# ChaissonLab/LRA

Hardware: AMD Instinct MI355X
Metric: aligned Gbp/s, 30 kb ONT vs GRCh38 (MapRead_lowacc end to end incl. SAM text), per job (higher is better)
Workload: dtype int32

## Files before the change

### lra_amd/csrc/aog.hip

```cpp
#include "common.h"
#include <stdlib.h>
#include <algorithm>
#include <vector>
#include <type_traits>

namespace {

constexpr int MISS = -(1 << 30);
enum { A_DONE = 0, A_LEFT = 1, A_DOWN = 2, A_DIAG = 3, A_BORDER = 4, A_GAPLEFT = 5, A_GAPDOWN = 6 };

constexpr int CLASS_A_BYTES = 10 * 1024;
constexpr int CLASS_B_BYTES = 64 * 1024;
constexpr int CLASS_M1_BYTES = 20 * 1024;
constexpr int CLASS_M2_BYTES = 32 * 1024;
constexpr int LN_MAX = 24, LN_ROWW = 2;
constexpr int LN_ARROW_WORDS = LN_MAX * LN_ROWW, LN_PREV_WORDS = LN_MAX + 2, LN_CODE_BYTES = LN_MAX + 1;
constexpr int LN_BYTES = 64 * (4 * LN_ARROW_WORDS + 4 * LN_PREV_WORDS + 2 * LN_CODE_BYTES);
constexpr int NCLS = 19;
constexpr int CLASS_S_BYTES = 2560;
constexpr long HBM_SLOT_BYTES = 4L << 20;
constexpr long HBM_SLOT_B_BYTES = 8L << 20;
constexpr int ROLL_WINDOW = 256;
constexpr int ROLL_CODE_BYTES = 4096;
constexpr int REG_S_BYTES = 2048, REG_M_BYTES = 8192, REG_L_BYTES = 32768;
constexpr int REG_L_USED = 16384;

__device__ __forceinline__ int code_n(unsigned char c) {
  if (c < 8) return c & 3;
  switch (c) {
    case 'A': case 'a': return 0;
    case 'C': case 'c': return 1;
    case 'G': case 'g': return 2;
    case 'T': case 't': return 3;
    default: return 4;
  }
}

struct Geo {
  int qLen, tLen, diag, k, R, qB, tB;
  bool top;
  int n;
  int nUsed;
};

__host__ __device__ __forceinline__ bool make_geo(int qLen, int tLen, int k0, Geo& g) {
  g.qLen = qLen; g.tLen = tLen;
  g.diag = max(1, min(qLen, tLen));
  int k = min(g.diag, k0);
  g.top = true;
  if (g.diag + 2 * k >= max(qLen, tLen)) { k *= 2; g.top = false; }
  g.k = k;
  g.R = 2 * k + 3;
  long n = (long)(3 + k + g.diag) * g.R;
  g.qB = min(g.diag + k, qLen + 1);
  g.tB = min(g.diag + k, tLen + 1);
  if (n > (1L << 28)) { g.n = 0; g.nUsed = 0; return false; }
  g.n = (int)n;
  g.nUsed = g.top ? g.n : min(g.n, g.tB * g.R);
  return true;
}

__host__ __device__ __forceinline__ long align4(long x) { return (x + 3) & ~3L; }

__host__ __device__ __forceinline__ long need_bytes(const Geo& g) {
  long suf = g.top ? (4L * g.n + align4(g.n)) : 0;
  return 4L * g.nUsed + align4(g.nUsed) + suf + 16L * (g.diag + 1) + align4(g.qLen + 1) + align4(g.tLen + 1);
}

__host__ __device__ __forceinline__ long need_bytes_reg(const Geo& g) { return align4(g.nUsed) + align4(g.qLen + 1) + align4(g.tLen + 1); }

struct Shape { int qLen, tLen, k0; };
struct Scoring { int m, mm, indel; };
template <typename P, typename S>
__host__ __device__ __forceinline__ bool problem_ok(const P& pr, const S& a, Geo& g) {
  bool ok = pr.qLen >= 0 && pr.tLen >= 0 && pr.k0 >= 1 && make_geo(pr.qLen, pr.tLen, pr.k0, g);
  long mx = max(abs(a.m), max(abs(a.mm), abs(a.indel)));
  return ok && ((long)(pr.qLen + pr.tLen + 16) * (mx + 1) < (1L << 28));
}

__host__ __device__ __forceinline__ int class_of(const Geo& g) {
  const long need = need_bytes(g);
  int cls = need <= CLASS_A_BYTES ? 0 : need <= CLASS_M1_BYTES ? 4 : need <= CLASS_M2_BYTES ? 5 : need <= CLASS_B_BYTES ? 1 : 2;
  if (g.k + 1 <= 32) cls = cls == 0 ? 7 : cls == 4 ? 8 : cls == 5 ? 9 : cls;
  if (need <= CLASS_S_BYTES && g.k + 1 <= 16) cls = 3;
  if (cls == 2 && need > HBM_SLOT_BYTES) cls = 6;
  if (cls == 6 && need > HBM_SLOT_B_BYTES) return -1;
  if (!g.top) {
    const long nr = need_bytes_reg(g);
    if (g.qLen <= LN_MAX && g.tLen <= LN_MAX) { const int mx = max(g.qLen, g.tLen); cls = mx <= 3 ? 14 : mx <= 6 ? 15 : mx <= 10 ? 16 : mx <= 16 ? 17 : 18; }
    else if (g.k + 2 <= 16 && nr <= REG_S_BYTES) cls = 10;
    else if (g.k + 2 <= 32 && nr <= REG_M_BYTES) cls = 11;
    else if (g.k + 2 <= 64 && nr <= REG_L_USED) cls = 12;
  }
  return cls;
}

__host__ __device__ __forceinline__ bool hbm_codes_in_lds(const Geo& g) { return g.qLen + g.tLen + 2 <= ROLL_CODE_BYTES; }
__host__ __device__ __forceinline__ bool hbm_in_regs(const Geo& g, int G) { return g.k + 2 <= G; }
__host__ __device__ __forceinline__ bool hbm_rolling(const Geo& g, int G) { return !g.top && (hbm_in_regs(g, G) || (2 * g.k + 3 <= ROLL_WINDOW && hbm_codes_in_lds(g))); }

__host__ __device__ __forceinline__ int path_of(const Geo& g, int cls) {
  int path = g.top ? LRA_AOG_PATH_SUFFIX : 0;
  if (cls == 2 || cls == 6) {
    const bool rolling = hbm_rolling(g, 64);
    path |= !rolling ? LRA_AOG_PATH_SCORES_HBM : hbm_in_regs(g, 64) ? LRA_AOG_PATH_SCORES_REGS : LRA_AOG_PATH_SCORES_ROLLING;
    if (rolling && hbm_codes_in_lds(g)) path |= LRA_AOG_PATH_CODES_LDS;
  } else {
    path |= (cls >= 10 && cls <= 12) ? LRA_AOG_PATH_SCORES_REGS : LRA_AOG_PATH_SCORES_LDS;
    path |= LRA_AOG_PATH_CODES_LDS;
  }
  return path;
}

struct Work {
  int* sPre; int* sSuf; int* loMax; int* loIdx; int* upMax; int* upIdx;
  signed char* pPre; signed char* pSuf; unsigned char* qc; unsigned char* tc;
};

template <typename BytePtr>
__device__ __forceinline__ Work carve(BytePtr base, const Geo& g) {
  Work w;
  auto* p = base;
  w.sPre = (int*)p; p += 4L * g.nUsed;
  w.sSuf = (int*)p; if (g.top) p += 4L * g.n;
  w.loMax = (int*)p; p += 4L * (g.diag + 1);
  w.loIdx = (int*)p; p += 4L * (g.diag + 1);
  w.upMax = (int*)p; p += 4L * (g.diag + 1);
  w.upIdx = (int*)p; p += 4L * (g.diag + 1);
  w.pPre = (signed char*)p; p += align4(g.nUsed);
  w.pSuf = (signed char*)p; if (g.top) p += align4(g.n);
  w.qc = (unsigned char*)p; p += align4(g.qLen + 1);
  w.tc = (unsigned char*)p;
  return w;
}

__device__ __forceinline__ void wave_sync() {
  __builtin_amdgcn_fence(__ATOMIC_RELEASE, "workgroup");
  __builtin_amdgcn_wave_barrier();
  __builtin_amdgcn_fence(__ATOMIC_ACQUIRE, "workgroup");
}

__device__ __forceinline__ void wave_sync_lds() {
  __builtin_amdgcn_fence(__ATOMIC_RELEASE, "wavefront");
  __builtin_amdgcn_wave_barrier();
  __builtin_amdgcn_fence(__ATOMIC_ACQUIRE, "wavefront");
}

struct Problem {
  const char* q; const char* t;
  int qLen, tLen, k0, m, mm, indel;
};

__device__ __forceinline__ int dpp_from_prev_lane(int v) { return __builtin_amdgcn_update_dpp(MISS, v, 0x138, 0xf, 0xf, false); }
__device__ __forceinline__ int dpp_from_next_lane(int v) { return __builtin_amdgcn_update_dpp(MISS, v, 0x130, 0xf, 0xf, false); }

template <int G, typename ArrowPtr, typename CodePtr>
__device__ __forceinline__ int reg_fill(int lane, int gbase, const Geo& g, int m, int mm, int indel, ArrowPtr P, CodePtr qc, CodePtr tc) {
  const int qLen = g.qLen, tLen = g.tLen, k = g.k, R = g.R, diag = g.diag, qB = g.qB, tB = g.tB;
  auto pre = [&](int i, int j) -> int {
    int v = MISS;
    if (j == 0 && i >= 1 && i < k + 1) v = indel * i;
    if (i == 0 && j >= 1 && j <= k + 1) v = indel * j;
    if (i == 0 && j == 0) v = 0;
    if (qLen >= tLen) { if (j == i + k + 1 && i <= diag - k - 1) v = MISS; if (i == j + k + 1 && j >= 1 && j < diag + k - 1) v = MISS; }
    if (qLen <= tLen) { if (i == j + k + 1 && j < diag - 1) v = MISS; if (j == i + k + 1 && j >= 1 && j < diag + k) v = MISS; }
    return v;
  };
  const int Wd = 2 * k + 3;
  const int sLast = max((qB - 1) + (tB - 1), 0);
  const int ci = qB - 1, cj = tB - 1;
  int vE = MISS, vO = MISS;
  const bool firstE = ((0 - k - 1) & 1) == 0;
  const int dE = 2 * lane - k - 1, dO = dE + 1;
  const bool okE = 2 * lane < Wd && dE >= -k && dE <= k, okO = 2 * lane + 1 < Wd && dO >= -k && dO <= k;
  const int sLoE = okE ? 2 + abs(dE) : INT_MAX, sHiE = min(2 * (qB - 1) - dE, 2 * (tB - 1) + dE);
  const int sLoO = okO ? 2 + abs(dO) : INT_MAX, sHiO = min(2 * (qB - 1) - dO, 2 * (tB - 1) + dO);
  const int s0E = firstE ? 0 : 1, s0O = firstE ? 1 : 0;
  int iE = (s0E + dE) >> 1, jE = s0E - iE, iO = (s0O + dO) >> 1, jO = s0O - iO;
  int adE = jE * R + 2 * lane, adO = jO * R + 2 * lane + 1;
  auto codes_match = [&](int i, int j) -> bool { return qc[min(max(i, 0), qLen)] == tc[min(max(j, 0), tLen)]; };
  bool eqE = codes_match(iE, jE), eqO = codes_match(iO, jO);
  auto step = [&](int s, auto isE) {
    constexpr bool E = decltype(isE)::value;
    const int nb1 = E ? dpp_from_prev_lane(vO) : dpp_from_next_lane(vE);
    const int i = E ? iE : iO, j = E ? jE : jO;
    const bool nxt = codes_match(i + 1, j + 1);
    int v = MISS;
    if (s >= (E ? sLoE : sLoO) && s <= (E ? sHiE : sHiO)) {
      const int sIns = (E ? nb1 : vE) + indel;
      const int sDel = (E ? vO : nb1) + indel;
      const int sMat = (E ? vE : vO) + ((E ? eqE : eqO) ? m : mm);
      const int best = max(sIns, max(sDel, sMat));
      v = best;
      P[E ? adE : adO] = (signed char)((best == sIns) ? A_LEFT : (best == sDel) ? A_DOWN : A_DIAG);
    } else if (s <= k + 1) {
      if (2 * lane + (E ? 0 : 1) < Wd && i >= 0 && j >= 0) v = pre(i, j);
    }
    if (E) { vE = v; eqE = nxt; iE++; jE++; adE += R; } else { vO = v; eqO = nxt; iO++; jO++; adO += R; }
  };
  int s = 0;
  bool lastE;
  if (firstE) {
    for (; s + 1 <= sLast; s += 2) { step(s, std::true_type{}); step(s + 1, std::false_type{}); }
    lastE = false;
    if (s <= sLast) { step(s, std::true_type{}); lastE = true; }
  } else {
    for (; s + 1 <= sLast; s += 2) { step(s, std::false_type{}); step(s + 1, std::true_type{}); }
    lastE = true;
    if (s <= sLast) { step(s, std::false_type{}); lastE = false; }
  }
  const int ddc = ci - cj + k + 1;
  const int corner = lastE ? vE : vO;
  return (ci >= 0 && cj >= 0 && ddc >= 0 && ddc < Wd && ((ddc & 1) == 0) == lastE) ? __shfl(corner, gbase + (ddc >> 1)) : MISS;
}

template <int G, typename BytePtr>
__device__ __forceinline__ void solve(int wlane, const Problem& pr, const Geo& g, BytePtr mem, int* out_score,
                      int* out_nb, int* blocks, long cap, int* out_status, int* roll = nullptr, int chunkBytes = 8192) {
  const int qLen = g.qLen, tLen = g.tLen, k = g.k, R = g.R, diag = g.diag, n = g.n, nUsed = g.nUsed;
  const int m = pr.m, mm = pr.mm, indel = pr.indel;
  const int lane = wlane & (G - 1), gbase = wlane - lane;
  Work w = carve(mem, g);
  int status = 0;
  auto PI = [&](int i, int j) { return j * R + (i - j) + k + 1; };
  auto inb = [&](int s) { return s >= 0 && s < n; };
#define PSET(slot, sc, ar)                                                         \
  do { int s__ = (slot); if (inb(s__)) { if (s__ < nUsed) { if (!rolling) w.sPre[s__] = (sc); w.pPre[s__] = (ar); } } else status |= LRA_ST_OOB_SLOT; } while (0)
#define SSET(slot, sc, ar)                                                         \
  do { int s__ = (slot); if (inb(s__)) { w.sSuf[s__] = (sc); w.pSuf[s__] = (ar); } else status |= LRA_ST_OOB_SLOT; } while (0)

  for (int x = lane; x <= qLen; x += G) w.qc[x] = x ? code_n((unsigned char)pr.q[x - 1]) : 0;
  for (int x = lane; x <= tLen; x += G) w.tc[x] = x ? code_n((unsigned char)pr.t[x - 1]) : 0;
  const bool codesInLds = hbm_codes_in_lds(g);
  const bool rolling = roll != nullptr && hbm_rolling(g, G);
  unsigned char* lq = (unsigned char*)(roll + 3 * ROLL_WINDOW); unsigned char* lt = lq + (qLen + 1);
  if (rolling && codesInLds) {
    for (int x = lane; x <= qLen; x += G) lq[x] = x ? code_n((unsigned char)pr.q[x - 1]) : 0;
    for (int x = lane; x <= tLen; x += G) lt[x] = x ? code_n((unsigned char)pr.t[x - 1]) : 0;
  }
  if (rolling) {
    const long head = min((long)nUsed, (long)((16 - ((uintptr_t)&w.pPre[0] & 15)) & 15));
    for (long x = lane; x < head; x += G) w.pPre[x] = -1;
    const long body = (nUsed - head) >> 4;
    int4* p16 = (int4*)(&w.pPre[0] + head);
    for (long x = lane; x < body; x += G) p16[x] = make_int4(-1, -1, -1, -1);
    for (long x = head + (body << 4) + lane; x < nUsed; x += G) w.pPre[x] = -1;
  }
  else for (int x = lane; x < nUsed; x += G) { w.sPre[x] = MISS; w.pPre[x] = -1; }
  if (g.top)
    for (int x = lane; x < n; x += G) { w.sSuf[x] = MISS; w.pSuf[x] = -1; }
  for (int x = lane; x <= diag; x += G) { w.loMax[x] = MISS; w.loIdx[x] = 0; w.upMax[x] = MISS; w.upIdx[x] = 0; }
  wave_sync();
  for (int i = 1 + lane; i < k + 1; i += G) PSET(PI(i, 0), indel * i, A_LEFT);
  for (int j = 1 + lane; j <= k + 1; j += G) PSET(PI(0, j), indel * j, A_DOWN);
  if (lane == 0) PSET(PI(0, 0), 0, A_DONE);
  wave_sync();
  if (qLen >= tLen) {
    for (int i = lane; i <= diag - k - 1; i += G) PSET(PI(i, i + k + 1), MISS, A_BORDER);
    for (int i = 1 + lane; i < diag + k - 1; i += G) PSET(PI(i + k + 1, i), MISS, A_BORDER);
  }
  if (qLen <= tLen) {
    for (int j = lane; j < diag - 1; j += G) PSET(PI(j + k + 1, j), MISS, A_BORDER);
    for (int j = 1 + lane; j < diag + k; j += G) PSET(PI(j - k - 1, j), MISS, A_BORDER);
  }
  wave_sync();
  const int qB = g.qB, tB = g.tB;
  int rollResult = MISS;
  if (rolling) {
    auto pre = [&](int i, int j) -> int {
      int v = MISS;
      if (j == 0 && i >= 1 && i < k + 1) v = indel * i;
      if (i == 0 && j >= 1 && j <= k + 1) v = indel * j;
      if (i == 0 && j == 0) v = 0;
      if (qLen >= tLen) { if (j == i + k + 1 && i <= diag - k - 1) v = MISS; if (i == j + k + 1 && j >= 1 && j < diag + k - 1) v = MISS; }
      if (qLen <= tLen) { if (i == j + k + 1 && j < diag - 1) v = MISS; if (j == i + k + 1 && j >= 1 && j < diag + k) v = MISS; }
      return v;
    };
    const int Wd = 2 * k + 3;
    const int sLast = (qB - 1) + (tB - 1);
    const bool inRegs = hbm_in_regs(g, G);
    if (inRegs) rollResult = codesInLds ? reg_fill<G>(lane, gbase, g, m, mm, indel, w.pPre, lq, lt) : reg_fill<G>(lane, gbase, g, m, mm, indel, w.pPre, w.qc, w.tc);
    for (int s = 0; !inRegs && s <= max(sLast, 0); s++) {
      int* cur = roll + (s % 3) * ROLL_WINDOW; const int* p1 = roll + ((s + 2) % 3) * ROLL_WINDOW; const int* p2 = roll + ((s + 1) % 3) * ROLL_WINDOW;
      int jlo = max(1, max(s - qB + 1, (s - k + 1) >> 1));
      if (s - k < 0) jlo = max(1, s - qB + 1);
      const int jhi = min(tB - 1, min(s - 1, (s + k) >> 1));
      for (int dd = lane; dd < Wd; dd += G) {
        const int d = dd - k - 1;
        int v = MISS;
        if (((s + d) & 1) == 0) {
          const int i = (s + d) >> 1, j = s - i;
          if (i >= 0 && j >= 0) {
            if (s >= 2 && j >= jlo && j <= jhi && d >= -k && d <= k) {
              const int sIns = p1[dd - 1] + indel, sDel = p1[dd + 1] + indel;
              const int sMat = p2[dd] + (lq[i] == lt[j] ? m : mm);
              const int best = max(sIns, max(sDel, sMat));
              const int ar = (best == sIns) ? A_LEFT : (best == sDel) ? A_DOWN : A_DIAG;
              v = best;
              w.pPre[PI(i, j)] = (signed char)ar;
            } else v = pre(i, j);
            if (i == qB - 1 && j == tB - 1) rollResult = v;
          }
        }
        cur[dd] = v;
      }
      wave_sync_lds();
    }
    wave_sync();
    if (!inRegs) { const int ddc = (qB - 1) - (tB - 1) + k + 1; rollResult = (ddc >= 0 && ddc < Wd) ? __shfl(rollResult, gbase + (ddc % G)) : MISS; }
  }
  for (int s = 2; !rolling && s <= (qB - 1) + (tB - 1); s++) {
    int jlo = max(1, max(s - qB + 1, (s - k + 1) >> 1));
    if (s - k < 0) jlo = max(1, s - qB + 1);
    int jhi = min(tB - 1, min(s - 1, (s + k) >> 1));
    for (int j = jlo + lane; j <= jhi; j += G) {
      int i = s - j;
      int sIns = w.sPre[PI(i - 1, j)] + indel;
      int sDel = w.sPre[PI(i, j - 1)] + indel;
      int sMat = w.sPre[PI(i - 1, j - 1)] + (w.qc[i] == w.tc[j] ? m : mm);
      int best = max(sIns, max(sDel, sMat));
      int ar = (best == sIns) ? A_LEFT : (best == sDel) ? A_DOWN : A_DIAG;
      int slot = PI(i, j);
      w.sPre[slot] = best;
      w.pPre[slot] = (signed char)ar;
    }
    wave_sync();
  }

  int ti, tj;
  int result;
  long nb = 0;
  const long iter_cap = 4L * (qLen + tLen + 8);
  int run = 0;
  auto flush = [&](int i_after, int j_after) {
    if (run > 0) {
      if (nb < cap) { blocks[3 * nb] = i_after; blocks[3 * nb + 1] = j_after; blocks[3 * nb + 2] = run; }
      else status |= LRA_ST_CAPACITY;
      nb++;
      run = 0;
    }
  };

  if (g.top) {
    for (int j = 1 + lane; j < tB && j <= diag; j += G) {
      int bm = MISS, bi = 0;
      int ihi = min(qB, j + k + 1);
      for (int i = max(1, j - k); i < ihi && i < qLen - k; i++) {
        int v = w.sPre[PI(i, j)];
        if (v >= bm) { bm = v; bi = i; }
      }
      w.loMax[j] = bm; w.loIdx[j] = bi;
    }
    for (int i = 1 + lane; i <= diag && i < qB; i += G) {
      int bm = MISS, bj = 0;
      int jhi = min(tB - 1, i + k);
      for (int j = max(1, i - k); j <= jhi && j < tLen; j++) {
        int v = w.sPre[PI(i, j)];
        if (v > bm) { bm = v; bj = j; }
      }
      w.upMax[i] = bm; w.upIdx[i] = bj;
    }
    if (lane == 0) {
      if (qLen >= tLen) { w.loMax[0] = 0; w.loIdx[0] = 0; }
      if (qLen <= tLen) { w.upMax[0] = 0; w.upIdx[0] = 0; }
    }
    wave_sync();
    const int qStart = max(0, qLen - diag);
    const int tStart = max(0, tLen - diag);
    const int tLow = max(0, tLen - diag - k - 1 - 1);
    const int qLow = max(0, qLen - diag - k - 1);
    const int tEnd = tLen + 1;
    auto SI = [&](int ii, int jj) {
      int a = ii - qLow, b = jj - tLow;
      return b * R + (a - b) + k + 1;
    };
    if (qLen >= tLen) {
      for (int i = qLow + lane; i < qStart + k + 1; i += G) SSET(SI(i, 0), w.loMax[0], A_GAPLEFT);
      wave_sync();
      for (int j = 1 + lane; j <= diag; j += G) SSET(SI(qLow + j - 1, j), w.loMax[j], A_GAPLEFT);
      wave_sync();
      for (int j = tStart + 1 + lane; j < tEnd - k; j += G) SSET(SI(qStart + (j - tStart - 1) + k + 1, j), MISS, A_BORDER);
      wave_sync();
    }
    if (qLen <= tLen) {
      for (int j = tLow + lane; j < tStart + k + 2; j += G) SSET(SI(qStart, j), w.upMax[0], A_GAPDOWN);
      wave_sync();
      for (int j = tStart + 1 + lane; j < tEnd; j += G) {
        int i = qStart + 1 + (j - tStart - 1);
        SSET(SI(i, j - k - 1), (i <= diag ? w.upMax[i] : MISS), A_GAPDOWN);
      }
      wave_sync();
      for (int j = tStart + lane; j < tEnd - k - 1; j += G) SSET(SI(qStart + (j - tStart), j + k + 1), MISS, A_BORDER);
      wave_sync();
    }
    const int c0 = qStart + diag - tLen;
    const bool qLong = qLen >= tLen;
    for (int s = (qLow + 1) + (tLow + 1); s <= qLen + tLen; s++) {
      int num = s - c0 - k;
      int jlo = (num >= 0) ? ((num + 1) >> 1) : -((-num) >> 1);
      jlo = max(jlo, max(tLow + 1, s - qLen));
      int num2 = s - c0 + k;
      int jhi = (num2 >= 0) ? (num2 >> 1) : -((-num2 + 1) >> 1);
      jhi = min(jhi, min(tLen, s - qLow - 1));
      for (int j = jlo + lane; j <= jhi; j += G) {
        int i = s - j;
        int delClose = MISS, insClose = MISS;
        if (qLong) delClose = (j <= diag) ? w.loMax[j] : MISS;
        else insClose = (i <= diag) ? w.upMax[i] : MISS;
        int a = SI(i - 1, j), b = SI(i, j - 1), c = SI(i - 1, j - 1);
        if (!inb(a) || !inb(b) || !inb(c)) { status |= LRA_ST_OOB_SLOT; continue; }
        int sIns = w.sSuf[a] + indel;
        int sDel = w.sSuf[b] + indel;
        int sMat = w.sSuf[c] + (w.qc[i] == w.tc[j] ? m : mm);
        int best = max(delClose, max(insClose, max(sIns, max(sDel, sMat))));
        int ar = (best == sIns) ? A_LEFT : (best == sDel) ? A_DOWN : (best == sMat) ? A_DIAG
                 : (best == delClose) ? A_GAPLEFT : A_GAPDOWN;
        SSET(SI(i, j), best, (signed char)ar);
      }
      wave_sync();
    }
    ti = qLen; tj = tLen;
    int s0 = SI(ti, tj);
    int arrow = inb(s0) ? w.pSuf[s0] : -1;
    result = inb(s0) ? w.sSuf[s0] : MISS;
    if (lane == 0) {
      long it = 0;
      while (arrow != A_DONE && arrow != A_GAPDOWN && arrow != A_GAPLEFT && ti >= 0 && tj >= 0) {
        if (++it > iter_cap) { status |= LRA_ST_NO_TERMINATION; break; }
        if (arrow == A_DIAG) { run++; ti--; tj--; }
        else if (arrow == A_LEFT) { flush(ti, tj); ti--; }
        else if (arrow == A_DOWN) { flush(ti, tj); tj--; }
        else { status |= LRA_ST_NO_TERMINATION; break; }
        if (ti >= 0 && tj >= 0) { int sl = SI(ti, tj); arrow = inb(sl) ? w.pSuf[sl] : -1; if (!inb(sl)) status |= LRA_ST_OOB_SLOT; }
      }
      flush(ti, tj);
      if (arrow == A_GAPDOWN && ti >= 0 && ti <= diag) tj = w.upIdx[ti];
      else if (arrow == A_GAPLEFT && tj >= 0 && tj <= diag) ti = w.loIdx[tj];
    }
  } else {
    ti = qB - 1; tj = tB - 1;
    result = rolling ? rollResult : w.sPre[PI(ti, tj)];
  }
  if (rolling) {
    unsigned char* chunk = (unsigned char*)(roll + 3 * ROLL_WINDOW + ROLL_CODE_BYTES / 4);
    const int chRows = max(1, chunkBytes / R);
    int cLo = 1, cHi = 0;
    auto arrowAt = [&](int i, int j) -> int {
      if (j < cLo || j > cHi) {
        cHi = j; cLo = max(0, j - chRows + 1);
        wave_sync();
        const long base = (long)cLo * R, len = (long)(cHi - cLo + 1) * R;
        for (long x = lane; x < len; x += G) chunk[x] = (unsigned char)w.pPre[base + x];
        wave_sync();
      }
      return (int)(signed char)chunk[(j - cLo) * R + (i - j) + k + 1];
    };
    auto flushL = [&](int i_after, int j_after) {
      if (run > 0) {
        if (nb < cap) { if (lane == 0) { blocks[3 * nb] = i_after; blocks[3 * nb + 1] = j_after; blocks[3 * nb + 2] = run; } }
        else status |= LRA_ST_CAPACITY;
        nb++;
        run = 0;
      }
    };
    constexpr int A_OFF = 100, A_WIN = 101;
    const unsigned long long gmask = (~0ULL >> (64 - G)) << gbase;
    if (ti >= 0 && tj >= 0 && inb(PI(ti, tj))) {
      while (true) {
        (void)arrowAt(ti, tj);
        const int jl = tj - lane;
        const bool on = ti - lane >= 0 && jl >= 0;
        const int a = !on ? A_OFF : jl < cLo ? A_WIN : (int)(signed char)chunk[(jl - cLo) * R + (ti - tj) + k + 1];
        const unsigned long long nd = (__ballot(a != A_DIAG) & gmask) >> gbase;
        const int f = nd ? __ffsll((long long)nd) - 1 : G;
        run += f; ti -= f; tj -= f;
        if (f == G) { if (ti < 0 || tj < 0) break; continue; }
        const int af = __shfl(a, gbase + f);
        if (af == A_WIN) continue;
        if (af == A_OFF) break;
        if (af == A_LEFT) { flushL(ti, tj); ti--; }
        else if (af == A_DOWN) { flushL(ti, tj); tj--; }
        else { if (af != A_BORDER && af != A_DONE && af != A_GAPLEFT && af != A_GAPDOWN) status |= LRA_ST_NO_TERMINATION; break; }
        if (ti < 0 || tj < 0) break;
      }
    }
    flushL(ti, tj);
  } else if (lane == 0) {
    int arrow = (ti >= 0 && tj >= 0 && inb(PI(ti, tj))) ? w.pPre[PI(ti, tj)] : A_DONE;
    long it = 0;
    while (arrow != A_BORDER && arrow != A_DONE && ti >= 0 && tj >= 0) {
      if (++it > iter_cap) { status |= LRA_ST_NO_TERMINATION; break; }
      if (arrow == A_DIAG) { run++; ti--; tj--; }
      else if (arrow == A_LEFT) { flush(ti, tj); ti--; }
      else if (arrow == A_DOWN) { flush(ti, tj); tj--; }
      else { if (arrow != A_GAPLEFT && arrow != A_GAPDOWN) status |= LRA_ST_NO_TERMINATION; break; }
      if (ti < 0 || tj < 0) break;
      arrow = w.pPre[PI(ti, tj)];
    }
    flush(ti, tj);
  }
#undef PSET
#undef SSET
  nb = __shfl(nb, gbase);
  int fi = __shfl(ti, gbase), fj = __shfl(tj, gbase);
  wave_sync();
  long nw = min(nb, cap);
  for (long x = lane; x < (nw + 1) / 2; x += G) {
    long y = nw - 1 - x;
    int a0 = blocks[3 * x], a1 = blocks[3 * x + 1], a2 = blocks[3 * x + 2];
    int b0 = blocks[3 * y], b1 = blocks[3 * y + 1], b2 = blocks[3 * y + 2];
    blocks[3 * x] = b0 - fi; blocks[3 * x + 1] = b1 - fj; blocks[3 * x + 2] = b2;
    if (y != x) { blocks[3 * y] = a0 - fi; blocks[3 * y + 1] = a1 - fj; blocks[3 * y + 2] = a2; }
  }
  for (int off = G / 2; off > 0; off >>= 1) status |= __shfl_xor(status, off);
  if (lane == 0) {
    int r = result;
    if (r < -(1 << 29)) r = (int)(unsigned int)((long)INT_MIN + ((long)r - (long)MISS));
    *out_score = r;
    *out_nb = (int)nb;
    *out_status = status;
  }
}

template <int G, typename BytePtr>
__device__ __forceinline__ void solve_reg(int wlane, const Problem& pr, const Geo& g, BytePtr mem, int* out_score, int* out_nb, int* blocks, long cap, int* out_status) {
  const int qLen = g.qLen, tLen = g.tLen, k = g.k, R = g.R, diag = g.diag, n = g.n, nUsed = g.nUsed;
  const int m = pr.m, mm = pr.mm, indel = pr.indel;
  const int lane = wlane & (G - 1), gbase = wlane - lane;
  auto* P = (signed char*)&mem[0];
  auto* qc = (unsigned char*)&mem[align4(nUsed)];
  auto* tc = (unsigned char*)&mem[align4(nUsed) + align4(qLen + 1)];
  int status = 0;
  auto PI = [&](int i, int j) { return j * R + (i - j) + k + 1; };
  auto inb = [&](int s_) { return s_ >= 0 && s_ < n; };
#define PSETA(slot, ar) do { int s__ = (slot); if (inb(s__)) { if (s__ < nUsed) P[s__] = (ar); } else status |= LRA_ST_OOB_SLOT; } while (0)
  for (int x = lane; x <= qLen; x += G) qc[x] = x ? code_n((unsigned char)pr.q[x - 1]) : 0;
  for (int x = lane; x <= tLen; x += G) tc[x] = x ? code_n((unsigned char)pr.t[x - 1]) : 0;
  { auto* P4 = (int*)&mem[0]; for (int x = lane; x < (int)(align4(nUsed) >> 2); x += G) P4[x] = -1; }
  wave_sync();
  for (int i = 1 + lane; i < k + 1; i += G) PSETA(PI(i, 0), A_LEFT);
  for (int j = 1 + lane; j <= k + 1; j += G) PSETA(PI(0, j), A_DOWN);
  if (lane == 0) PSETA(PI(0, 0), A_DONE);
  wave_sync();
  if (qLen >= tLen) {
    for (int i = lane; i <= diag - k - 1; i += G) PSETA(PI(i, i + k + 1), A_BORDER);
    for (int i = 1 + lane; i < diag + k - 1; i += G) PSETA(PI(i + k + 1, i), A_BORDER);
  }
  if (qLen <= tLen) {
    for (int j = lane; j < diag - 1; j += G) PSETA(PI(j + k + 1, j), A_BORDER);
    for (int j = 1 + lane; j < diag + k; j += G) PSETA(PI(j - k - 1, j), A_BORDER);
// ... 187 lines not shown
    solve_reg<G>(lane, pr, g, smem + (wave_in_wg * GPW + lane / G) * BYTES, &a.score[p], &a.nblocks[p], blk, cap, &a.status[p]);
    wave_sync();
  }
}



template <int MX>
__global__ void __launch_bounds__(64) aog_lane_kernel(BatchArgs a, int cls) {
  constexpr int LN_MAX = MX, LN_ROWW = MX > 16 ? 2 : 1;
  constexpr int LN_ARROW_WORDS = LN_MAX * LN_ROWW, LN_PREV_WORDS = LN_MAX + 2, LN_CODE_BYTES = LN_MAX + 1;
  constexpr int LN_BYTES = 64 * (4 * LN_ARROW_WORDS + 4 * LN_PREV_WORDS + 2 * LN_CODE_BYTES);
  __shared__ __attribute__((aligned(16))) char smem[LN_BYTES];
  const int lane = threadIdx.x;
  unsigned* AR = (unsigned*)smem;
  int* PV = (int*)(smem + 64 * 4 * LN_ARROW_WORDS);
  unsigned char* QC = (unsigned char*)(smem + 64 * 4 * (LN_ARROW_WORDS + LN_PREV_WORDS));
  unsigned char* TC = QC + 64 * LN_CODE_BYTES;
  const int count = a.counts[cls];
  for (int x0 = blockIdx.x * 64; x0 < count; x0 += gridDim.x * 64) {
    const int x = x0 + lane;
    if (x < count) {
      const int p = a.list[a.offs[cls] + x];
      Problem pr; Geo g; int ok;
      load_problem(a, p, pr, g, ok);
      const int qLen = g.qLen, tLen = g.tLen, k = g.k, diag = g.diag, qB = g.qB, tB = g.tB;
      const int m = pr.m, mm = pr.mm, indel = pr.indel;
      {
        unsigned char cq[LN_MAX], ct[LN_MAX];
#pragma unroll
        for (int i = 0; i < LN_MAX; i++) { cq[i] = i < qLen ? (unsigned char)pr.q[i] : 0; ct[i] = i < tLen ? (unsigned char)pr.t[i] : 0; }
#pragma unroll
        for (int i = 0; i < LN_MAX; i++) { QC[(i + 1) * 64 + lane] = (unsigned char)code_n(cq[i]); TC[(i + 1) * 64 + lane] = (unsigned char)code_n(ct[i]); }
      }
      auto in_region = [&](int i, int j) { return i >= 1 && i <= qB - 1 && j >= 1 && j <= tB - 1 && i - j <= k && j - i <= k; };
      auto pre = [&](int i, int j) -> int {
        int v = MISS;
        if (j == 0 && i >= 1 && i < k + 1) v = indel * i;
        if (i == 0 && j >= 1 && j <= k + 1) v = indel * j;
        if (i == 0 && j == 0) v = 0;
        if (qLen >= tLen) { if (j == i + k + 1 && i <= diag - k - 1) v = MISS; if (i == j + k + 1 && j >= 1 && j < diag + k - 1) v = MISS; }
        if (qLen <= tLen) { if (i == j + k + 1 && j < diag - 1) v = MISS; if (j == i + k + 1 && j >= 1 && j < diag + k) v = MISS; }
        return v;
      };
      auto pre_arrow = [&](int i, int j) -> int {
        int v = -1;
        if (i < 0 || j < 0) return v;
        if (j == 0 && i >= 1 && i < k + 1) v = A_LEFT;
        if (i == 0 && j >= 1 && j <= k + 1) v = A_DOWN;
        if (i == 0 && j == 0) v = A_DONE;
        if (qLen >= tLen) { if (j == i + k + 1 && i <= diag - k - 1) v = A_BORDER; if (i == j + k + 1 && j >= 1 && j < diag + k - 1) v = A_BORDER; }
        if (qLen <= tLen) { if (i == j + k + 1 && j < diag - 1) v = A_BORDER; if (j == i + k + 1 && j >= 1 && j < diag + k) v = A_BORDER; }
        return v;
      };
      for (int j = 1; j <= tB - 1; j++) {
        const int ilo = max(1, j - k), ihi = min(qB - 1, j + k);
        const int tcj = TC[j * 64 + lane];
        int left = pre(ilo - 1, j);
        int dg = in_region(ilo - 1, j - 1) ? PV[(ilo - 1) * 64 + lane] : pre(ilo - 1, j - 1);
        unsigned long long acc = 0;
        const int hi2 = j >= 2 ? min(qB - 1, j - 1 + k) : 0;
        for (int i = ilo; i <= ihi; i++) {
          int up;
          if (i <= hi2) up = PV[i * 64 + lane];
          else up = (j == 1 && i < k + 1) ? indel * i : MISS;
          const int sIns = left + indel, sDel = up + indel, sMat = dg + (QC[i * 64 + lane] == tcj ? m : mm);
          const int best = max(sIns, max(sDel, sMat));
          const int ar = (best == sIns) ? A_LEFT : (best == sDel) ? A_DOWN : A_DIAG;
          acc |= (unsigned long long)ar << (2 * (i - ilo));
          PV[i * 64 + lane] = best;
          dg = up; left = best;
        }
        AR[((j - 1) * LN_ROWW) * 64 + lane] = (unsigned)acc; if (LN_ROWW > 1) AR[((j - 1) * LN_ROWW + 1) * 64 + lane] = (unsigned)(acc >> 32);
      }
      const int ci = qB - 1, cj = tB - 1;
      const int result = in_region(ci, cj) ? PV[ci * 64 + lane] : ((ci >= 0 && cj >= 0) ? pre(ci, cj) : MISS);
      auto arrow_at = [&](int i, int j) -> int {
        if (!in_region(i, j)) return pre_arrow(i, j);
        const int sh = 2 * (i - max(1, j - k));
        const unsigned w = AR[((j - 1) * LN_ROWW + (LN_ROWW > 1 ? (sh >> 5) : 0)) * 64 + lane];
        return (int)((w >> (sh & 31)) & 3u);
      };
      const long cap = (long)(a.block_off[p + 1] - a.block_off[p]);
      int* blocks = a.blocks + 3 * a.block_off[p];
      int status = 0;
      long nb = 0; int fi = ci, fj = cj;
      for (int pass = 0; pass < 2; pass++) {
        const long nw = min(nb, cap);
        long w = 0; int run = 0; int ti = ci, tj = cj;
        auto flush = [&](int i_after, int j_after) {
          if (run > 0) {
            if (pass == 1 && w < nw) { int* b = blocks + 3 * (nw - 1 - w); b[0] = i_after - fi; b[1] = j_after - fj; b[2] = run; }
            w++; run = 0;
          }
        };
        int arrow = (ti >= 0 && tj >= 0) ? arrow_at(ti, tj) : A_DONE;
        while (arrow != A_BORDER && arrow != A_DONE && ti >= 0 && tj >= 0) {
          if (arrow == A_DIAG) { run++; ti--; tj--; }
          else if (arrow == A_LEFT) { flush(ti, tj); ti--; }
          else if (arrow == A_DOWN) { flush(ti, tj); tj--; }
          else { if (arrow != A_GAPLEFT && arrow != A_GAPDOWN) status |= LRA_ST_NO_TERMINATION; break; }
          if (ti < 0 || tj < 0) break;
          arrow = arrow_at(ti, tj);
        }
        flush(ti, tj);
        if (pass == 0) { nb = w; fi = ti; fj = tj; if (nb > cap) status |= LRA_ST_CAPACITY; }
      }
      int r = result;
      if (r < -(1 << 29)) r = (int)(unsigned int)((long)INT_MIN + ((long)r - (long)MISS));
      a.score[p] = r; a.nblocks[p] = (int)nb; a.status[p] = status;
    }
  }
}

}

int lra_aog_launch_device(lra_ctx* ctx, int n, const char* d_qseq, const char* d_tseq, const uint64_t* d_q_off,
                          const int32_t* d_q_len, const uint64_t* d_t_off, const int32_t* d_t_len, const int32_t* d_k,
                          int m, int mm, int indel, int32_t* d_score, int32_t* d_nblocks, int32_t* d_blocks,
                          const uint64_t* d_block_off, int32_t* d_status) {
  if (!ctx) return LRA_ERR_INVALID;
  if (n < 0) return lra_set_err(ctx, LRA_ERR_INVALID, "n < 0");
  if (n == 0) return LRA_OK;
  LRA_HIP_CHECK(ctx, hipSetDevice(ctx->device));
  BatchArgs a;
  a.n = n; a.qseq = d_qseq; a.tseq = d_tseq; a.q_off = d_q_off; a.q_len = d_q_len; a.t_off = d_t_off; a.t_len = d_t_len;
  a.k = d_k; a.m = m; a.mm = mm; a.indel = indel;
  a.score = d_score; a.nblocks = d_nblocks; a.blocks = d_blocks; a.block_off = d_block_off; a.status = d_status;
  char* s0 = (char*)lra_scratch(ctx, 0, 384 + sizeof(int) * (size_t)n + (size_t)n + 64);
  if (!s0) return LRA_ERR_NOMEM;
  a.counts = (int*)s0; a.offs = a.counts + 32; a.cursor = a.counts + 64; a.list = (int*)(s0 + 384); a.cls8 = (unsigned char*)(a.list + n);
  const int perCu = ctx->pipelined ? 6 : 8;
  a.gslots = ctx->num_cu * perCu; a.gslot_bytes = HBM_SLOT_BYTES;
  a.chunk_bytes = 8192;
  a.gslotsB = ctx->num_cu; a.gslotB_bytes = HBM_SLOT_B_BYTES;
  a.gscratch = (char*)lra_scratch(ctx, 1, (size_t)a.gslots * a.gslot_bytes + (size_t)a.gslotsB * a.gslotB_bytes);
  if (!a.gscratch) return LRA_ERR_NOMEM;
  a.gscratchB = a.gscratch + (size_t)a.gslots * a.gslot_bytes;
  if (getenv("LRA_AOG_DBG")) {
    std::vector<int32_t> hq(n), ht(n), hk(n);
    (void)hipMemcpy(hq.data(), d_q_len, (size_t)n * 4, hipMemcpyDeviceToHost); (void)hipMemcpy(ht.data(), d_t_len, (size_t)n * 4, hipMemcpyDeviceToHost);
    (void)hipMemcpy(hk.data(), d_k, (size_t)n * 4, hipMemcpyDeviceToHost);
    long nTop = 0, nBigK = 0, steps = 0; long byNeed[8] = {0, 0, 0, 0, 0, 0, 0, 0}; long byK[4] = {0, 0, 0, 0}; long cellsBy[8] = {0, 0, 0, 0, 0, 0, 0, 0};
    for (int p = 0; p < n; p++) {
      const int q = hq[p], t = ht[p]; const int diag = std::max(1, std::min(q, t)); int k = std::min(diag, hk[p]); bool top = true;
      if (diag + 2 * k >= std::max(q, t)) { k *= 2; top = false; }
      const long R = 2 * k + 3, tB = std::min(diag + k, t + 1); const long nU = top ? (3 + k + diag) * R : std::min((3 + k + diag) * R, tB * R);
      if (top) { nTop++; continue; }
      if (k > 62) { nBigK++; continue; }
      const long need = nU + q + t + 8;
      const int b = need <= 2048 ? 0 : need <= 4096 ? 1 : need <= 8192 ? 2 : need <= 16384 ? 3 : need <= 32768 ? 4 : need <= 65536 ? 5 : need <= 160 * 1024 ? 6 : 7;
      byNeed[b]++; cellsBy[b] += nU; steps += q + t;
      byK[k <= 14 ? 0 : k <= 30 ? 1 : k <= 62 ? 2 : 3]++;
    }
    fprintf(stderr, "[aog] n %d top %ld k>62 %ld | arrows+codes <=2K %ld <=4K %ld <=8K %ld <=16K %ld <=32K %ld <=64K %ld <=160K %ld more %ld | cells(M) %.1f %.1f %.1f %.1f %.1f %.1f %.1f %.1f | k<=14 %ld <=30 %ld <=62 %ld | steps(M) %.1f\n",
            n, nTop, nBigK, byNeed[0], byNeed[1], byNeed[2], byNeed[3], byNeed[4], byNeed[5], byNeed[6], byNeed[7], cellsBy[0] / 1e6, cellsBy[1] / 1e6, cellsBy[2] / 1e6, cellsBy[3] / 1e6,
            cellsBy[4] / 1e6, cellsBy[5] / 1e6, cellsBy[6] / 1e6, cellsBy[7] / 1e6, byK[0], byK[1], byK[2], steps / 1e6);
  }
  LRA_HIP_CHECK(ctx, hipMemsetAsync(a.counts, 0, 384, ctx->stream));
  const int cblocks = (int)(((long)n + CLS_ITEMS * 1024 - 1) / (CLS_ITEMS * 1024));
  hipLaunchKernelGGL(aog_classify, dim3(cblocks), dim3(1024), 0, ctx->stream, a);
  hipLaunchKernelGGL(aog_offsets, dim3(1), dim3(64), 0, ctx->stream, a);
  hipLaunchKernelGGL(aog_scatter, dim3(cblocks), dim3(1024), 0, ctx->stream, a);
  int wgA = min((n + 3) / 4, ctx->num_cu * 5);
  int wgB = min(n, ctx->num_cu * 2);
  int wgC = min(n, a.gslots);
  LRA_HIP_CHECK(ctx, hipFuncSetAttribute((const void*)aog_kernel<7>, hipFuncAttributeMaxDynamicSharedMemorySize, 8 * CLASS_A_BYTES));
  LRA_HIP_CHECK(ctx, hipFuncSetAttribute((const void*)aog_kernel<1>, hipFuncAttributeMaxDynamicSharedMemorySize, CLASS_B_BYTES));
  LRA_HIP_CHECK(ctx, hipFuncSetAttribute((const void*)aog_kernel<9>, hipFuncAttributeMaxDynamicSharedMemorySize, 2 * CLASS_M2_BYTES));
  const hipStream_t sm = ctx->stream;
  const hipStream_t s1 = lra_side_fork(ctx, 1), s2 = lra_side_fork(ctx, 2), s3 = lra_side_fork(ctx, 3);
  lra_time_begin(ctx, "aog_lds_large", s1);
  hipLaunchKernelGGL(aog_kernel<1>, dim3(wgB), dim3(64), CLASS_B_BYTES, s1, a);
  lra_time_end(ctx, s1);
  lra_time_begin(ctx, "aog_lds_small", s2);
  hipLaunchKernelGGL(aog_kernel<7>, dim3(min((n + 7) / 8, ctx->num_cu * 2)), dim3(256), 8 * CLASS_A_BYTES, s2, a);
  hipLaunchKernelGGL(aog_kernel<0>, dim3(wgA), dim3(256), 4 * CLASS_A_BYTES, s2, a);
  lra_time_end(ctx, s2);
  lra_time_begin(ctx, "aog_lds_tiny", s2);
  hipLaunchKernelGGL(aog_kernel<3>, dim3(min((n + 15) / 16, ctx->num_cu * 8)), dim3(256), 16 * CLASS_S_BYTES, s2, a);
  lra_time_end(ctx, s2);
  lra_time_begin(ctx, "aog_lds_medium", s3);
  hipLaunchKernelGGL(aog_kernel<8>, dim3(min((n + 1) / 2, ctx->num_cu * 4)), dim3(64), 2 * CLASS_M1_BYTES, s3, a);
  hipLaunchKernelGGL(aog_kernel<9>, dim3(min((n + 1) / 2, ctx->num_cu * 2)), dim3(64), 2 * CLASS_M2_BYTES, s3, a);
  hipLaunchKernelGGL(aog_kernel<4>, dim3(min(n, ctx->num_cu * 8)), dim3(64), CLASS_M1_BYTES, s3, a);
  hipLaunchKernelGGL(aog_kernel<5>, dim3(min(n, ctx->num_cu * 5)), dim3(64), CLASS_M2_BYTES, s3, a);
  lra_time_end(ctx, s3);
  lra_time_begin(ctx, "aog_lane");
  const int nb64 = (n + 63) / 64;
  hipLaunchKernelGGL(aog_lane_kernel<24>, dim3(min(nb64, ctx->num_cu * 7)), dim3(64), 0, sm, a, 18);
  hipLaunchKernelGGL(aog_lane_kernel<16>, dim3(min(nb64, ctx->num_cu * 14)), dim3(64), 0, sm, a, 17);
  hipLaunchKernelGGL(aog_lane_kernel<10>, dim3(min(nb64, ctx->num_cu * 22)), dim3(64), 0, sm, a, 16);
  hipLaunchKernelGGL(aog_lane_kernel<6>, dim3(min(nb64, ctx->num_cu * 32)), dim3(64), 0, sm, a, 15);
  hipLaunchKernelGGL(aog_lane_kernel<3>, dim3(min(nb64, ctx->num_cu * 32)), dim3(64), 0, sm, a, 14);
  lra_time_end(ctx);
  lra_time_begin(ctx, "aog_reg");
  hipLaunchKernelGGL(aog_reg_kernel<10>, dim3(min((n + 15) / 16, ctx->num_cu * 10)), dim3(256), 16 * REG_S_BYTES, sm, a);
  lra_time_end(ctx);
  lra_time_begin(ctx, "aog_reg_medium", s2);
  hipLaunchKernelGGL(aog_reg_kernel<11>, dim3(min((n + 3) / 4, ctx->num_cu * 10)), dim3(128), 4 * REG_M_BYTES, s2, a);
  lra_time_end(ctx, s2);
  lra_time_begin(ctx, "aog_reg_large", s3);
  hipLaunchKernelGGL(aog_reg_kernel<12>, dim3(min(n, ctx->num_cu * 10)), dim3(64), REG_L_USED, s3, a);
  lra_time_end(ctx, s3);
  lra_time_begin(ctx, "aog_hbm");
  hipLaunchKernelGGL(aog_kernel<2>, dim3(wgC), dim3(64), 3 * ROLL_WINDOW * 4 + ROLL_CODE_BYTES + a.chunk_bytes, sm, a);
  hipLaunchKernelGGL(aog_kernel<6>, dim3(min(n, a.gslotsB)), dim3(64), 3 * ROLL_WINDOW * 4 + ROLL_CODE_BYTES + a.chunk_bytes, sm, a);
  lra_time_end(ctx);
  lra_side_join(ctx, 1); lra_side_join(ctx, 2); lra_side_join(ctx, 3);
  LRA_HIP_CHECK(ctx, hipGetLastError());
  return LRA_OK;
}

extern "C" int lra_affine_one_gap_align_batch(lra_ctx* ctx, int n, const char* d_qseq, const char* d_tseq,
                                              const uint64_t* d_q_off, const int32_t* d_q_len,
                                              const uint64_t* d_t_off, const int32_t* d_t_len,
                                              const int32_t* d_k, int m, int mm, int indel,
                                              int32_t* d_score, int32_t* d_nblocks, int32_t* d_blocks,
                                              const uint64_t* d_block_off, int32_t* d_status) {
  return lra_aog_launch_device(ctx, n, d_qseq, d_tseq, d_q_off, d_q_len, d_t_off, d_t_len, d_k, m, mm, indel, d_score, d_nblocks,
                               d_blocks, d_block_off, d_status);
}

extern "C" int lra_aog_class_of_batch(int n, const int32_t* q_len, const int32_t* t_len, const int32_t* k, int m, int mm, int indel,
                                      int32_t* cls_out, int32_t* path_out) {
  if (n < 0 || (n > 0 && (!q_len || !t_len || !k || !cls_out || !path_out))) return LRA_ERR_INVALID;
  const Scoring sc = {m, mm, indel};
  for (int p = 0; p < n; p++) {
    Geo g;
    const Shape sh = {q_len[p], t_len[p], k[p]};
    const int cls = problem_ok(sh, sc, g) ? class_of(g) : -1;
    cls_out[p] = cls;
    path_out[p] = cls < 0 ? 0 : path_of(g, cls);
  }
  return LRA_OK;
}
```

Measured before the change: 1.086.

## Fill two-band prefix and suffix DP in registers with DPP wavefront

For two-band (top) alignment problems that fit the register path, the prefix band is now filled with the register-resident anti-diagonal kernel, which also stores scores. A new suf_fill does the same for the suffix band, including the gap-close terms. These replace the per-anti-diagonal loops that went through memory and needed a wave sync at every step. It adds complex index and boundary logic that must reproduce the old border conditions exactly, plus a debug stats print.

```diff
diff --git a/lra_amd/csrc/aog.hip b/lra_amd/csrc/aog.hip
--- a/lra_amd/csrc/aog.hip
+++ b/lra_amd/csrc/aog.hip
@@ -154,8 +154,8 @@
 __device__ __forceinline__ int dpp_from_prev_lane(int v) { return __builtin_amdgcn_update_dpp(MISS, v, 0x138, 0xf, 0xf, false); }
 __device__ __forceinline__ int dpp_from_next_lane(int v) { return __builtin_amdgcn_update_dpp(MISS, v, 0x130, 0xf, 0xf, false); }
 
-template <int G, typename ArrowPtr, typename CodePtr>
-__device__ __forceinline__ int reg_fill(int lane, int gbase, const Geo& g, int m, int mm, int indel, ArrowPtr P, CodePtr qc, CodePtr tc) {
+template <int G, typename ArrowPtr, typename CodePtr, typename ScorePtr = std::nullptr_t>
+__device__ __forceinline__ int reg_fill(int lane, int gbase, const Geo& g, int m, int mm, int indel, ArrowPtr P, CodePtr qc, CodePtr tc, ScorePtr S = nullptr) {
   const int qLen = g.qLen, tLen = g.tLen, k = g.k, R = g.R, diag = g.diag, qB = g.qB, tB = g.tB;
   auto pre = [&](int i, int j) -> int {
     int v = MISS;
@@ -193,6 +193,7 @@
       const int best = max(sIns, max(sDel, sMat));
       v = best;
       P[E ? adE : adO] = (signed char)((best == sIns) ? A_LEFT : (best == sDel) ? A_DOWN : A_DIAG);
+      if constexpr (!std::is_same<ScorePtr, std::nullptr_t>::value) S[E ? adE : adO] = best;
     } else if (s <= k + 1) {
       if (2 * lane + (E ? 0 : 1) < Wd && i >= 0 && j >= 0) v = pre(i, j);
     }
@@ -212,6 +213,67 @@
   const int ddc = ci - cj + k + 1;
   const int corner = lastE ? vE : vO;
   return (ci >= 0 && cj >= 0 && ddc >= 0 && ddc < Wd && ((ddc & 1) == 0) == lastE) ? __shfl(corner, gbase + (ddc >> 1)) : MISS;
+}
+
+template <int G, typename CodePtr>
+__device__ __forceinline__ void suf_fill(int lane, const Geo& g, int m, int mm, int indel, const Work& w, CodePtr qc, CodePtr tc) {
+  const int qLen = g.qLen, tLen = g.tLen, k = g.k, R = g.R, diag = g.diag;
+  const bool qLong = qLen >= tLen;
+  const int qLow = qLong ? qLen - tLen - k - 1 : 0, tLow = qLong ? 0 : tLen - qLen - k - 2;
+  const int base = (qLen - tLen) - k - 1;
+  const int* cl = qLong ? w.loMax : w.upMax;
+  const int cl0 = cl[0];
+  const int s00 = qLow + tLow, sLast = qLen + tLen;
+  const bool firstE = ((s00 - base) & 1) == 0;
+  const int eE = 2 * lane, eO = eE + 1, dE = eE + base, dO = eO + base;
+  const bool okE = eE >= 1 && eE <= 2 * k + 1, okO = eO <= 2 * k + 1;
+  const int sLoE = okE ? max(2 * (tLow + 1) + dE, 2 * (qLow + 1) - dE) : INT_MAX, sHiE = min(2 * tLen + dE, 2 * qLen - dE);
+  const int sLoO = okO ? max(2 * (tLow + 1) + dO, 2 * (qLow + 1) - dO) : INT_MAX, sHiO = min(2 * tLen + dO, 2 * qLen - dO);
+  const int s0E = firstE ? s00 : s00 + 1, s0O = firstE ? s00 + 1 : s00;
+  int iE = (s0E + dE) >> 1, jE = s0E - iE, iO = (s0O + dO) >> 1, jO = s0O - iO;
+  int adE = (jE - tLow) * R + (iE - qLow) - (jE - tLow) + k + 1, adO = (jO - tLow) * R + (iO - qLow) - (jO - tLow) + k + 1;
+  const int railHi = eE == 2 * k + 2 ? 1 : 0;
+  auto codes_match = [&](int i, int j) -> bool { return qc[min(max(i, 0), qLen)] == tc[min(max(j, 0), tLen)]; };
+  auto close_at = [&](int i, int j, int rail) -> int { return cl[min(max(qLong ? j + rail : i, 0), diag)]; };
+  bool eqE = codes_match(iE, jE), eqO = codes_match(iO, jO);
+  int xE = close_at(iE, jE, railHi), xO = close_at(iO, jO, 0);
+  int vE = MISS, vO = MISS;
+  auto step = [&](int s, auto isE) {
+    constexpr bool E = decltype(isE)::value;
+    const int nb1 = E ? dpp_from_prev_lane(vO) : dpp_from_next_lane(vE);
+    const int i = E ? iE : iO, j = E ? jE : jO, e = E ? eE : eO, x = E ? xE : xO;
+    const bool nxt = codes_match(i + 1, j + 1);
+    const int nxtX = close_at(i + 1, j + 1, E ? railHi : 0);
+    int v = MISS;
+    if (s >= (E ? sLoE : sLoO) && s <= (E ? sHiE : sHiO)) {
+      const int delClose = qLong ? x : MISS, insClose = qLong ? MISS : x;
+      const int sIns = (E ? nb1 : vE) + indel;
+      const int sDel = (E ? vO : nb1) + indel;
+      const int sMat = (E ? vE : vO) + ((E ? eqE : eqO) ? m : mm);
+      const int best = max(delClose, max(insClose, max(sIns, max(sDel, sMat))));
+      const int ar = (best == sIns) ? A_LEFT : (best == sDel) ? A_DOWN : (best == sMat) ? A_DIAG : (best == delClose) ? A_GAPLEFT : A_GAPDOWN;
+      v = best;
+      w.sSuf[E ? adE : adO] = best; w.pSuf[E ? adE : adO] = (signed char)ar;
+    } else if (e <= 2 * k + 2) {
+      if (qLong) {
+        if (j == 0 && e <= 2 * k + 1) v = cl0;
+        if (e == 2 * k + 2 && j >= 0 && j <= diag - 1) v = x;
+      } else {
+        if ((i == 0 && j >= tLow + 1) || (e == 0 && j == tLow + 1)) v = cl0;
+        if (e == 2 * k + 2 && i >= 1 && i <= qLen) v = x;
+        if (e == 0 && i >= 0 && i <= qLen - k - 1) v = MISS;
+      }
+    }
+    if (E) { vE = v; eqE = nxt; xE = nxtX; iE++; jE++; adE += R; } else { vO = v; eqO = nxt; xO = nxtX; iO++; jO++; adO += R; }
+  };
+  int s = s00;
+  if (firstE) {
+    for (; s + 1 <= sLast; s += 2) { step(s, std::true_type{}); step(s + 1, std::false_type{}); }
+    if (s <= sLast) step(s, std::true_type{});
+  } else {
+    for (; s + 1 <= sLast; s += 2) { step(s, std::false_type{}); step(s + 1, std::true_type{}); }
+    if (s <= sLast) step(s, std::false_type{});
+  }
 }
 
 template <int G, typename BytePtr>
@@ -233,8 +295,9 @@
   for (int x = lane; x <= tLen; x += G) w.tc[x] = x ? code_n((unsigned char)pr.t[x - 1]) : 0;
   const bool codesInLds = hbm_codes_in_lds(g);
   const bool rolling = roll != nullptr && hbm_rolling(g, G);
+  const bool preRegs = g.top && hbm_in_regs(g, G);
   unsigned char* lq = (unsigned char*)(roll + 3 * ROLL_WINDOW); unsigned char* lt = lq + (qLen + 1);
-  if (rolling && codesInLds) {
+  if ((rolling || (preRegs && roll != nullptr)) && codesInLds) {
     for (int x = lane; x <= qLen; x += G) lq[x] = x ? code_n((unsigned char)pr.q[x - 1]) : 0;
     for (int x = lane; x <= tLen; x += G) lt[x] = x ? code_n((unsigned char)pr.t[x - 1]) : 0;
   }
@@ -245,6 +308,10 @@
     int4* p16 = (int4*)(&w.pPre[0] + head);
     for (long x = lane; x < body; x += G) p16[x] = make_int4(-1, -1, -1, -1);
     for (long x = head + (body << 4) + lane; x < nUsed; x += G) w.pPre[x] = -1;
+  }
+  else if (preRegs) {
+    int* p4 = (int*)&w.pPre[0];
+    for (int x = lane; x < (int)(align4(nUsed) >> 2); x += G) p4[x] = -1;
   }
   else for (int x = lane; x < nUsed; x += G) { w.sPre[x] = MISS; w.pPre[x] = -1; }
   if (g.top)
@@ -309,7 +376,12 @@
     wave_sync();
     if (!inRegs) { const int ddc = (qB - 1) - (tB - 1) + k + 1; rollResult = (ddc >= 0 && ddc < Wd) ? __shfl(rollResult, gbase + (ddc % G)) : MISS; }
   }
-  for (int s = 2; !rolling && s <= (qB - 1) + (tB - 1); s++) {
+  if (preRegs) {
+    if (roll != nullptr && codesInLds) (void)reg_fill<G>(lane, gbase, g, m, mm, indel, w.pPre, lq, lt, w.sPre);
+    else (void)reg_fill<G>(lane, gbase, g, m, mm, indel, w.pPre, w.qc, w.tc, w.sPre);
+    wave_sync();
+  }
+  for (int s = 2; !rolling && !preRegs && s <= (qB - 1) + (tB - 1); s++) {
     int jlo = max(1, max(s - qB + 1, (s - k + 1) >> 1));
     if (s - k < 0) jlo = max(1, s - qB + 1);
     int jhi = min(tB - 1, min(s - 1, (s + k) >> 1));
@@ -395,7 +467,13 @@
     }
     const int c0 = qStart + diag - tLen;
     const bool qLong = qLen >= tLen;
-    for (int s = (qLow + 1) + (tLow + 1); s <= qLen + tLen; s++) {
+    const bool sufRegs = preRegs && qLen >= 1 && tLen >= 1;
+    if (sufRegs) {
+      if (roll != nullptr && codesInLds) suf_fill<G>(lane, g, m, mm, indel, w, lq, lt);
+      else suf_fill<G>(lane, g, m, mm, indel, w, w.qc, w.tc);
+      wave_sync();
+    }
+    for (int s = (qLow + 1) + (tLow + 1); !sufRegs && s <= qLen + tLen; s++) {
       int num = s - c0 - k;
       int jlo = (num >= 0) ? ((num + 1) >> 1) : -((-num) >> 1);
       jlo = max(jlo, max(tLow + 1, s - qLen));
@@ -889,6 +967,23 @@
       const int b = need <= 2048 ? 0 : need <= 4096 ? 1 : need <= 8192 ? 2 : need <= 16384 ? 3 : need <= 32768 ? 4 : need <= 65536 ? 5 : need <= 160 * 1024 ? 6 : 7;
       byNeed[b]++; cellsBy[b] += nU; steps += q + t;
       byK[k <= 14 ? 0 : k <= 30 ? 1 : k <= 62 ? 2 : 3]++;
+    }
+    {
+      long cnt[NCLS] = {0}, stp[NCLS] = {0}, reg[NCLS] = {0}, regStp[NCLS] = {0}, longest[NCLS] = {0};
+      const Scoring sc = {m, mm, indel};
+      for (int p = 0; p < n; p++) {
+        Geo g; const Shape sh = {hq[p], ht[p], hk[p]};
+        if (!problem_ok(sh, sc, g) || !g.top) continue;
+        const int cls = class_of(g);
+        if (cls < 0) continue;
+        const int qLow = std::max(0, g.qLen - g.diag - g.k - 1), tLow = std::max(0, g.tLen - g.diag - g.k - 2);
+        const long st = std::max(0, (g.qB - 1) + (g.tB - 1) - 1) + std::max(0, g.qLen + g.tLen - (qLow + tLow + 2) + 1);
+        const int G = cls == 3 ? 16 : cls >= 7 ? 32 : 64;
+        cnt[cls]++; stp[cls] += st; longest[cls] = std::max(longest[cls], st);
+        if (hbm_in_regs(g, G)) { reg[cls]++; regStp[cls] += st; }
+      }
+      for (int c = 0; c < NCLS; c++)
+        if (cnt[c]) fprintf(stderr, "[aog] two-band class %d: %ld problems, %ld steps (longest %ld); in registers %ld problems, %ld steps\n", c, cnt[c], stp[c], longest[c], reg[c], regStp[c]);
     }
     fprintf(stderr, "[aog] n %d top %ld k>62 %ld | arrows+codes <=2K %ld <=4K %ld <=8K %ld <=16K %ld <=32K %ld <=64K %ld <=160K %ld more %ld | cells(M) %.1f %.1f %.1f %.1f %.1f %.1f %.1f %.1f | k<=14 %ld <=30 %ld <=62 %ld | steps(M) %.1f\n",
             n, nTop, nBigK, byNeed[0], byNeed[1], byNeed[2], byNeed[3], byNeed[4], byNeed[5], byNeed[6], byNeed[7], cellsBy[0] / 1e6, cellsBy[1] / 1e6, cellsBy[2] / 1e6, cellsBy[3] / 1e6,
```

Result: slower. 1.062 (-2.2%).
